# clancylian/retinaface

Hardware: NVIDIA H100
Metric: faces/sec (end-to-end detect) (higher is better)
Workload: dtype f16

## Files before the change

### retinaface_b200/csrc/engine_internal.cuh

```cuda
#pragma once
#include <algorithm>
#include <cstdarg>
#include <cstdio>
#include <cstring>
#include <functional>
#include <map>
#include <memory>
#include <string>
#include <type_traits>
#include <vector>

#include "align.cuh"
#include "common.cuh"
#include "host_copy.h"
#include "model.h"
#include "postproc.cuh"
#include "preprocess.cuh"

using namespace rf;

#define RF_STR2(x) #x
#define RF_STR(x) RF_STR2(x)

namespace rf_eng {

// ... 234 lines not shown
    virtual void heads(const HeadsNode &n) = 0;
    virtual SegOut segment(const SegNode &s, int in);
    virtual void merge_aggr(const MergeNode &m);
    virtual void ssh(const SshNode &n);
};
void walk_network(PlanOps &ops);
struct StemPack { std::vector<float> w0, wd, wp; };
StemPack pack_stem(const StemNode &n);
std::vector<float> pack_dw(const FoldedConv &dw, float scale = 1.f);
struct DwGeom { int rows, nsplit, Rmax; };
DwGeom dw_geometry(int C, int N, int IH, int IW, int S, const std::function<bool(int rows, int N, int R)> &fits);
int dw2d_tile_w(rf_handle h, int C, int oh, int ow, int nsplit);
bool aggr_fits_one_wave(rf_handle h, int fh, int fw);

constexpr int TC_SMEM_LIMIT = 200 * 1024;
template <typename T>
void build_plan(rf_handle h);
cudaError_t tc_init();
template <typename OutT>
int plan_stem_fused(Builder &B, const StemNode &n, const char *suffix, float out_scale);
int resident_ctas(rf_handle h, const void *kern, int threads, size_t smem);
struct PersistentGrid { int run, grid; };
inline PersistentGrid persistent_grid(int tiles, int resident) {
    const int run = std::max(1, (tiles + resident - 1) / std::max(resident, 1));
    return {run, (tiles + run - 1) / run};
}
int plan_pair_tc(Builder &B, const PairNode &p, int in);
void plan_conv_tc(Builder &B, const ConvNode &c);
int plan_fpn_merge_h2(Builder &B, const MergeNode &m);
template <typename T>
void plan_heads(Builder &B, const HeadsNode &n, const float scale[3], const char *prefix, bool with_heads);
std::vector<__half> pack_tc_weights(const std::vector<const FoldedConv *> &cs, std::vector<float> &bias, int &Kpad, int nsplit = 1);
void build_plan_tiles(rf_handle h);
cudaError_t tile_init();
std::string describe_chains(rf_handle h);
void comm_release(rf_handle h);
void comm_wait_in_graph(rf_handle h, const Ctx &c, int n, cudaStream_t s);
int jpeg_info(rf_handle h, const uint8_t *data, size_t len, int *w, int *hgt);
int jpeg_decode(rf_handle h, const uint8_t *const *data, const size_t *len, int n, uint8_t *const *dst, const int *w, const int *hgt, cudaStream_t s);
void jpeg_release(rf_handle h);
const char *jpeg_backend(rf_handle h);
void build_plan_i8(rf_handle h);
cudaError_t tc_init_i8();

int check_n(rf_handle h, int n);
int check_frames(rf_handle h, const char *who, const rf_yuv_frame *frames, int n, int matrix);
int check_orientations(rf_handle h, const char *who, const int *orientations, int n);
void upload_plane(rf_handle h, cudaStream_t s, uint8_t *d_dst, const uint8_t *src, size_t row_bytes, size_t pitch, int rows);
int align_setup(rf_handle h, const char *who, const rf_align_params *p, AlignArgs &a);
// ... 86 lines not shown
```

### retinaface_b200/csrc/plan_fp.cu

```cuda
#include "engine_internal.cuh"
#include "kernels_simt.cuh"
#include "stem_tc.cuh"
#include "tc_conv.cuh"
#include "tc_dwpw2d.cuh"

namespace rf_eng {

#define CK_L(...) CK(launch_k(__VA_ARGS__))

std::vector<float> pack_gemm(const std::vector<const FoldedConv *> &cs, std::vector<float> &bias) {
    const int cin = cs[0]->cin, k = cs[0]->k;
    int N = 0;
    for (auto c : cs) N += c->cout;
    std::vector<float> w((size_t)k * k * cin * N);
    bias.assign(N, 0.f);
    int n0 = 0;
    for (auto c : cs) {
        for (int o = 0; o < c->cout; o++) {
            bias[n0 + o] = c->b[o];
            for (int ci = 0; ci < cin; ci++)
                for (int t = 0; t < k * k; t++)
                    w[((size_t)t * cin + ci) * N + n0 + o] = c->w[((size_t)o * cin + ci) * k * k + t];
        }
        n0 += c->cout;
// ... 54 lines not shown
}
void launch_tc_dwpw(const TcDwArgs &a_in, int nsplit, cudaStream_t s) {
    TcDwArgs a = a_in;
    a.mul_Wp = fast_div_mul((uint32_t)a.Wp); a.mul_Hp = fast_div_mul((uint32_t)a.Hp);
    a.mul_OW = fast_div_mul((uint32_t)a.OW); a.mul_OH = fast_div_mul((uint32_t)a.OH);
    const long M = (long)a.nimg * a.OH * a.OW;
    dim3 grid((unsigned)((M + a.rows - 1) / a.rows), nsplit);
    const size_t smem = tc_dw_smem_bytes(a);
    switch (tc_n_bucket(a.N)) {
        case 32: CK_L(k_tc_dwpw_staged<32>, grid, dim3(TC_THREADS), smem, s, a); break;
        case 64: CK_L(k_tc_dwpw_staged<64>, grid, dim3(TC_THREADS), smem, s, a); break;
        case 128: CK_L(k_tc_dwpw_staged<128>, grid, dim3(TC_THREADS), smem, s, a); break;
        default: CK_L(k_tc_dwpw_staged<256>, grid, dim3(TC_THREADS), smem, s, a); break;
    }
}
static void (*dw2d_kernel(int N))(TcDw2dArgs) {
    switch (tc_n_bucket(N)) {
        case 32: return k_tc_dwpw_2d<32>;
        case 64: return k_tc_dwpw_2d<64>;
        case 128: return k_tc_dwpw_2d<128>;
        default: return k_tc_dwpw_2d<256>;
    }
}
void launch_tc_dwpw_2d(TcDw2dArgs a, int resident, cudaStream_t s) {
    const PersistentGrid pg = persistent_grid(a.tiles_x * a.tiles_y * a.nimg, resident);
    a.run = pg.run;
    CK_L(dw2d_kernel(a.N), dim3((unsigned)pg.grid), dim3(TC_THREADS), tc_dw2d_smem_bytes(a), s, a);
}

int resident_ctas(rf_handle h, const void *kern, int threads, size_t smem) {
    if (!h->on_device) return h->num_sms;
    int per_sm = 0;
    CK(cudaOccupancyMaxActiveBlocksPerMultiprocessor(&per_sm, kern, threads, smem));
    if (per_sm < 1) throw PlanFail{RF_ERR_UNSUPPORTED, fmt("a kernel with %zu bytes of dynamic shared memory does not fit an SM", smem)};
    return per_sm * h->num_sms;
}

cudaError_t tc_init() {
    cudaError_t e;
#define RF_TC_ATTR(K_) if ((e = cudaFuncSetAttribute(K_, cudaFuncAttributeMaxDynamicSharedMemorySize, TC_SMEM_LIMIT))) return e
    RF_TC_ATTR((k_tc_conv_staged<32, false>)); RF_TC_ATTR((k_tc_conv_staged<64, false>)); RF_TC_ATTR((k_tc_conv_staged<128, false>)); RF_TC_ATTR((k_tc_conv_staged<256, false>));
    RF_TC_ATTR((k_tc_conv_staged<32, true>)); RF_TC_ATTR((k_tc_conv_staged<64, true>)); RF_TC_ATTR((k_tc_conv_staged<128, true>)); RF_TC_ATTR((k_tc_conv_staged<256, true>));
    RF_TC_ATTR(k_tc_dwpw_staged<32>); RF_TC_ATTR(k_tc_dwpw_staged<64>); RF_TC_ATTR(k_tc_dwpw_staged<128>); RF_TC_ATTR(k_tc_dwpw_staged<256>);
    RF_TC_ATTR(k_tc_dwpw_2d<32>); RF_TC_ATTR(k_tc_dwpw_2d<64>); RF_TC_ATTR(k_tc_dwpw_2d<128>); RF_TC_ATTR(k_tc_dwpw_2d<256>);
#undef RF_TC_ATTR
    return cudaSuccess;
}

static std::vector<__half> make_stem_blob(const StemPack &p, const std::vector<float> &b0, const std::vector<float> &bd, const std::vector<float> &bp) {
    std::vector<__half> b0img(2 * 4 * 16 * 8, __float2half(0.f)), b1img(2 * 16 * 8, __float2half(0.f));
    for (int k = 0; k < 27; k++)
        for (int o = 0; o < 8; o++) {
            const float wv = p.w0[k * 8 + o];
            const __half hi = __float2half(wv);
            b0img[((k / 8) * 16 + o) * 8 + (k % 8)] = hi;
            b0img[((4 + k / 8) * 16 + o) * 8 + (k % 8)] = __float2half(wv - __half2float(hi));
        }
    for (int c = 0; c < 8; c++)
// ... 25 lines not shown
        TcDwArgs a{};
        a.C = C; a.Rmax = R; a.Kpad = (C + 15) / 16 * 16; a.N = Ns; a.rows = rows;
        return R <= TC_MAX_R && tc_dw_smem_bytes(a) <= (size_t)TC_SMEM_LIMIT;
    });
    if (geo.rows == 0) throw PlanFail{RF_ERR_UNSUPPORTED, fmt("layer %s (%dx%d, %d channels) does not fit shared memory", dw.name.c_str(), iw, ih, C)};
    std::vector<float> bias;
    int Kpad = 0;
    std::vector<__half> img = pack_tc_weights({&pw}, bias, Kpad, geo.nsplit);
    size_t oimg = B.add_weights_h(img), obp = B.add_weights(bias);
    int tpw = B.tensor(p.out, oh, ow_, N);
    Step s;
    s.name = fmt("tc_dw%d+pw%d_s%d_%dto%d", i, i + 1, S, C, N);
    s.in = {tin}; s.out = {tpw};
    s.flops_per_img = 2.0 * oh * ow_ * C * 9 + 2.0 * oh * ow_ * C * N;
    s.bytes_per_img = ((double)ih * iw * C + (double)oh * ow_ * N) * es;
    const int tw = dw2d_tile_w(h, C, oh, ow_, geo.nsplit);
    TcDw2dArgs g2{};
    int resident = 0;
    if (tw) {
        s.name = fmt("tc2d_dw%d+pw%d_s%d_%dto%d", i, i + 1, S, C, N);
        g2.C = C; g2.IH = ih; g2.IW = iw; g2.OH = oh; g2.OW = ow_; g2.S = S; g2.N = N;
        g2.TH = 8; g2.TW = tw;
        tc_dw2d_finish(g2);
        resident = resident_ctas(h, (const void *)dw2d_kernel(N), TC_THREADS, tc_dw2d_smem_bytes(g2));
    }
    s.launch = [=](const Run &r) {
        if (tw) {
            TcDw2dArgs a = g2;
            a.in = T_(r, tin); a.nimg = r.n;
            a.wimg = h->d_weights_h + oimg; a.bias = Wd(obp); a.dw_w = Wd(owd); a.dw_b = Wd(obd); a.out = T_(r, tpw);
            launch_tc_dwpw_2d(a, resident, r.stream);
            return;
        }
        TcDwArgs a{};
        a.in = T_(r, tin); a.C = C; a.nimg = r.n; a.IH = ih; a.IW = iw; a.OH = oh; a.OW = ow_; a.S = S;
        a.N = N / geo.nsplit; a.Ntotal = N; a.Kpad = Kpad; a.rows = geo.rows; a.Wp = iw + 2; a.Hp = ih + 1; a.Rmax = geo.Rmax;
        a.wimg = h->d_weights_h + oimg; a.bias = Wd(obp); a.dw_w = Wd(owd); a.dw_b = Wd(obd); a.out = T_(r, tpw);
        launch_tc_dwpw(a, geo.nsplit, r.stream);
    };
    B.step(std::move(s));
    return tpw;
}

void plan_conv_tc(Builder &B, const ConvNode &c) {
    rf_handle h = B.h;
    const Model &m = h->model;
// ... 273 lines not shown
```

### retinaface_b200/csrc/plan_tile.cu

```cuda
#include <cstdlib>

#include "engine_internal.cuh"
#include "tile_chain.cuh"

namespace rf_eng {

namespace {

typedef CUresult (*EncodeTiledFn)(CUtensorMap *, CUtensorMapDataType, cuuint32_t, void *, const cuuint64_t *, const cuuint64_t *,
                                  const cuuint32_t *, const cuuint32_t *, CUtensorMapInterleave, CUtensorMapSwizzle, CUtensorMapL2promotion,
                                  CUtensorMapFloatOOBfill);
EncodeTiledFn g_encode = nullptr;

constexpr int TCH_SMEM_LIMIT = 226 * 1024;

CUtensorMap make_map(const void *base, int C, int W, int H, int n, int bc, int bw, int bh, int es) {
    CUtensorMap m;
    cuuint64_t dims[4] = {(cuuint64_t)C, (cuuint64_t)W, (cuuint64_t)H, (cuuint64_t)n};
    cuuint64_t strides[3] = {(cuuint64_t)C * 2, (cuuint64_t)W * C * 2, (cuuint64_t)H * W * C * 2};
    cuuint32_t box[4] = {(cuuint32_t)bc, (cuuint32_t)bw, (cuuint32_t)bh, 1};
    cuuint32_t est[4] = {1, (cuuint32_t)es, (cuuint32_t)es, 1};
    const CUtensorMapSwizzle sw = bc * 2 == 128 ? CU_TENSOR_MAP_SWIZZLE_128B : (bc * 2 == 64 ? CU_TENSOR_MAP_SWIZZLE_64B : CU_TENSOR_MAP_SWIZZLE_32B);
    CUresult r = g_encode(&m, CU_TENSOR_MAP_DATA_TYPE_FLOAT16, 4, const_cast<void *>(base), dims, strides, box, est, CU_TENSOR_MAP_INTERLEAVE_NONE, sw,
                          CU_TENSOR_MAP_L2_PROMOTION_L2_128B, CU_TENSOR_MAP_FLOAT_OOB_FILL_NONE);
    if (r != CUDA_SUCCESS) throw PlanFail{RF_ERR_CUDA, fmt("cuTensorMapEncodeTiled failed (%d) for a %dx%dx%d tensor, box %dx%dx%d", (int)r, C, W, H, bc, bw, bh)};
    return m;
}

int round_up(int v, int a) { return (v + a - 1) / a * a; }

}

struct TileChain {
    struct LBuf {
        int C = 0;
        int halo = 0;
        bool stored = false;
        int store_tensor = -1;
        int first = 1 << 30, last = -1;
        bool is_input = false, is_merge = false;
    };
    struct LStage {
        int type = TCH_CONV, Cin = 0, N = 0, taps = 1, stride = 1, in_buf = 0;
        std::vector<int> ob_buf, ob_c16, ob_relu;
        std::vector<__half> wd_img, wp_img;
// ... 317 lines not shown
            fprintf(stderr, "TRACE %s:", c.name.c_str());
            for (unsigned i = 0; i < n; i++) fprintf(stderr, " %llu@%llu", it->second[1 + 2 * i], it->second[2 + 2 * i] - it->second[2]);
            fprintf(stderr, "\n");
        }
        memset(it->second, 0, 8 * 1024);
        a.trace = it->second;
    }
#endif
    a.warena = reinterpret_cast<const unsigned char *>(h->d_weights_h);
    a.bias = h->d_weights + c.bias_off;
    TchMaps maps;
    memset(&maps, 0, sizeof maps);
    const TchBuf &b0 = a.buf[0];
    const int bc = std::min(c.in_C, 64);
    auto T_ = [&](int id) { return r.ctx.arena + h->tensors[id].offset; };
    if (c.in_s2) maps.in = make_map(T_(c.in_tensor), c.in_C, c.in_W, c.in_H, n, bc, 2 * a.Wl, 2 * b0.nrows, 2);
    else maps.in = make_map(T_(c.in_tensor), c.in_C, c.in_W, c.in_H, n, bc, a.Wl, b0.nrows, 1);
    if (c.merge_tensor >= 0) maps.aux = make_map(T_(c.merge_tensor), 64, c.W / 2, c.H / 2, n, 64, c.W / 2 + 2, a.merge_rows, 1);
    for (int i = 0; i < c.nstores; i++) maps.st[i] = make_map(T_(c.bufs[c.store_buf_of[i]].store_tensor), c.store_C[i], c.W, c.H, n, std::min(c.store_C[i], 64), c.W, 1, 1);
    if (c.level >= 0) {
        a.head.lv = h->lv[c.level];
        a.head.pb = r.ctx.pb;
        a.head.params = r.ctx.d_params;
        a.head.net_w = h->cfg.net_w; a.head.net_h = h->cfg.net_h;
        a.head.done = r.ctx.pb.tile_done;
        a.head.expected = (c.fused_nms && !r.single) ? h->tile_expected : 0;
        for (int k = 0; k < 3; k++) a.head.blobs[k] = r.blobs ? r.blobs[3 * c.level + k] : nullptr;
    }
    const int grid = std::min(a.ntiles, h->num_sms);
    CK(launch_k(k_tile_chain<0>, dim3((unsigned)grid), dim3(TCH_THREADS), (size_t)a.smem_bytes, st, maps, a));
}

void add_chain_step(Builder &B, std::shared_ptr<TileChain> c, int lane, double bytes_per_img) {
    rf_handle h = B.h;
// ... 16 lines not shown
}

std::string describe_chains(rf_handle h) {
    std::string out;
    for (auto &cp : h->chains) {
        const TileChain &c = *cp;
        const TchArgs &a = c.args;
        out += fmt("%s: %dx%d map, TH=%d HT=%d Wl=%d, %d tiles/image, %d stages, %d MMA tiles/tile, smem %d B (%s weights), stores %d\n",
                   c.name.c_str(), c.W, c.H, a.TH, a.HT, a.Wl, a.tiles_per_img, a.nstages, c.mtiles, a.smem_bytes, a.resident ? "resident" : "streamed",
                   c.nstores);
    }
    return out;
}

cudaError_t tile_init() {
    if (!g_encode) {
        void *fn = nullptr;
        cudaDriverEntryPointQueryResult q;
        cudaError_t e = cudaGetDriverEntryPoint("cuTensorMapEncodeTiled", &fn, cudaEnableDefault, &q);
        if (e != cudaSuccess) return e;
        if (!fn) return cudaErrorNotSupported;
        g_encode = (EncodeTiledFn)fn;
    }
    return cudaFuncSetAttribute(k_tile_chain<0>, cudaFuncAttributeMaxDynamicSharedMemorySize, TCH_SMEM_LIMIT);
}

enum { TM_A = 1, TM_B = 2, TM_C = 4, TM_D = 8, TM_E = 16, TM_AGGR = 32, TM_SSH = 64, TM_HEAD = 128, TM_NMS = 256, TM_ALL = 511 };
constexpr unsigned TM_LATENCY = TM_SSH | TM_HEAD | TM_NMS;
constexpr unsigned TM_LATENCY_SMALL = TM_AGGR | TM_SSH | TM_HEAD | TM_NMS;
constexpr unsigned TM_THROUGHPUT = 0;

struct TileOps : PlanOps {
    unsigned mask;
    const bool single = env_int("RF_TILE_SINGLE", 0) != 0;
    std::shared_ptr<TileChain> ssh_chain[3];
    bool split_heads = false;
    TileOps(rf_handle h, unsigned m) : PlanOps(h), mask(m) {
        if (!(mask & TM_SSH)) mask &= ~(TM_HEAD | TM_NMS);
// ... 122 lines not shown
```

### retinaface_b200/csrc/tc_dwpw2d.cuh

```cuda
#pragma once
#include "tc_conv.cuh"

namespace rf {

struct TcDw2dArgs {
    const __half *in;
    int C, nimg, IH, IW, OH, OW, S;
    int N;
    int TH, TW;
    int tiles_x, tiles_y;
    int run;
    int PH, PW;
    uint32_t lbo_a;
    uint32_t mul_TW, mul_tiles_x, mul_tiles;
    const __half *wimg;
    const float *bias;
    const float *dw_w, *dw_b;
    __half *out;
};

inline void tc_dw2d_finish(TcDw2dArgs &a) {
    const int G = a.C >> 3;
    a.PH = (a.TH - 1) * a.S + 3;
    a.PW = (a.TW - 1) * a.S + 3;
    a.tiles_x = (a.OW + a.TW - 1) / a.TW;
    a.tiles_y = (a.OH + a.TH - 1) / a.TH;
    a.lbo_a = (uint32_t)(128 + 8 / G) * 16;
    a.mul_TW = fast_div_mul((uint32_t)a.TW);
    a.mul_tiles_x = fast_div_mul((uint32_t)a.tiles_x);
    a.mul_tiles = fast_div_mul((uint32_t)(a.tiles_x * a.tiles_y));
}
inline size_t tc_dw2d_smem_bytes(const TcDw2dArgs &a) {
    return 2 * (size_t)a.PH * a.PW * a.C * 2 + (size_t)(a.C / 8) * a.lbo_a + (size_t)a.C * a.N * 2 + 128;
}

#ifndef RF_DW2D_OCC
#define RF_DW2D_OCC 3
#endif
template <int NT>
__global__ void __launch_bounds__(TC_THREADS, RF_DW2D_OCC) k_tc_dwpw_2d(const TcDw2dArgs a) {
    extern __shared__ __align__(128) unsigned char smem[];
    __shared__ __align__(8) uint64_t bar_b;
    __shared__ float s_bias[256];
    __shared__ __align__(16) float s_dww[9 * 64];
    __shared__ __align__(16) float s_dwb[64];

    const int tid = threadIdx.x, warp = tid >> 5, lane = tid & 31;
    const int G = a.C >> 3, lg = 31 - __clz(G);
    const int PH = a.PH, PW = a.PW;
    const uint32_t lbo_a = a.lbo_a;
    const int pix = a.C * 2;
    const uint32_t stage_bytes = (uint32_t)(PH * PW * pix);
    unsigned char *sA = smem + 2 * (size_t)stage_bytes;
    unsigned char *sB = sA + (size_t)G * lbo_a;
    const int tiles = a.tiles_x * a.tiles_y;
    const int t_end = min((int)blockIdx.x * a.run + a.run, tiles * a.nimg);
    auto decode = [&](int t, int &b, int &oy0, int &ox0) {
        b = fast_div(t, a.mul_tiles);
        const int trem = t - b * tiles, ty0 = fast_div(trem, a.mul_tiles_x);
        oy0 = ty0 * a.TH; ox0 = (trem - ty0 * a.tiles_x) * a.TW;
    };

    if (tid == 0) {
        tc::mbar_init(&bar_b, 1);
        asm volatile("fence.mbarrier_init.release.cluster;" ::: "memory");
        const unsigned bytes = (unsigned)((size_t)a.C * a.N * 2);
        tc::mbar_expect_tx(&bar_b, bytes);
        tc::bulk_g2s(sB, a.wimg, bytes, &bar_b);
    }
    pdl_trigger();
    if (tid < a.N) s_bias[tid] = a.bias[tid];
    for (int i = tid; i < 9 * a.C; i += TC_THREADS) s_dww[i] = dw_weight_f16(a.dw_w[i]);
    if (tid < a.C) s_dwb[tid] = a.dw_b[tid];
    pdl_wait();
    const uint32_t sS_s = tc::smem_u32(smem);
    auto stage = [&](int t, int buf) {
        int b, oy0, ox0;
        decode(t, b, oy0, ox0);
        const int iy0 = oy0 * a.S - 1, ix0 = ox0 * a.S - 1;
        const int per_row = PW << lg;
        const int px_lo = max(0, -ix0), px_hi = min(PW, a.IW - ix0);
        const unsigned px_n = (unsigned)max(px_hi - px_lo, 0);
        for (int py = warp; py < PH; py += TC_THREADS / 32) {
            const int iy = iy0 + py;
            const bool rowok = iy >= 0 && iy < a.IH;
            const __half *src_row = a.in + (ptrdiff_t)(((b * a.IH + (rowok ? iy : 0)) * a.IW + ix0) * a.C);
            const uint32_t dst_row = sS_s + (uint32_t)buf * stage_bytes + (uint32_t)(py * PW * pix);
            const __half *zsrc = a.in;
            for (int i = lane; i < per_row; i += 32) {
                const bool ok = rowok && (unsigned)((i >> lg) - px_lo) < px_n;
                cp_async16_zfill_s(dst_row + (uint32_t)i * 16u, ok ? src_row + i * 8 : zsrc, ok);
            }
        }
        cp_async_commit();
    };
    auto stencil = [&](auto s_, const unsigned char *sS) {
        constexpr int S = decltype(s_)::value;
        const int items = a.TH * (a.TW >> 1) << lg;
        for (int it = tid; it < items; it += TC_THREADS) {
            const int g = it & (G - 1), rest = it >> lg;
            const int ty = fast_div(2 * rest, a.mul_TW), tx = 2 * rest - ty * a.TW;
            float acc[1][2][8];
            dw_bias8(acc[0][0], &s_dwb[g * 8]);
#pragma unroll
            for (int i = 0; i < 8; i++) acc[0][1][i] = acc[0][0][i];
            dw_stencil_block<S, 1, 2>(acc, sS + (ty * S * PW + tx * S) * pix + g * 16, PW * pix, pix, &s_dww[g * 8], a.C);
            unsigned char *dst = sA + (size_t)g * lbo_a + (size_t)(ty * a.TW + tx) * 16;
            *reinterpret_cast<uint4 *>(dst) = dw_relu_h8(acc[0][0]);
            *reinterpret_cast<uint4 *>(dst + 16) = dw_relu_h8(acc[0][1]);
        }
    };
    const int rows = a.TH * a.TW;
    const bool has_gemm = 64 * (warp >> 2) < rows;
    const int t_begin = (int)blockIdx.x * a.run;
    stage(t_begin, 0);
    for (int t = t_begin; t < t_end; t++) {
        const int buf = (t - t_begin) & 1;
        cp_async_wait_all();
        __syncthreads();
        if (t + 1 < t_end) stage(t + 1, buf ^ 1);
        const unsigned char *sS = smem + (size_t)buf * stage_bytes;
        if (a.S == 1) stencil(std::integral_constant<int, 1>{}, sS);
        else stencil(std::integral_constant<int, 2>{}, sS);
        tc::fence_async_smem();
        __syncthreads();
        if (!has_gemm) continue;
        tc::mbar_wait(&bar_b, 0);
        int b, oy0, ox0;
        decode(t, b, oy0, ox0);
        long orow[2];
#pragma unroll
        for (int e = 0; e < 2; e++) {
            const int r = tc_frag_row() + 8 * e;
            const int ty = fast_div(r, a.mul_TW), tx = r - ty * a.TW;
            const int oy = oy0 + ty, ox = ox0 + tx;
            orow[e] = (r < rows && oy < a.OH && ox < a.OW) ? (long)((b * a.OH + oy) * a.OW + ox) : -1;
        }
        const uint32_t a_addr = tc::smem_u32(sA) + (uint32_t)(64 * (warp >> 2)) * 16u, b_addr = tc::smem_u32(sB);
        const uint32_t lbo_b = (uint32_t)a.N * 16;
        const TcOut o{a.out, a.N, a.N, 1, nullptr, 0, 0};
        wg::for_chunks<(NT < 32 ? NT : 32)>(a.N, [&](auto nc, int n0) {
            constexpr int NC = decltype(nc)::value;
            float d[NC / 2];
            wg::fence();
            wg::mma_ss<NC>(d, wg::desc(a_addr, lbo_a, 128), wg::desc(b_addr + (uint32_t)n0 * 16u, lbo_b, 128), 0);
            for (int ks = 1; ks < (a.C >> 4); ks++) {
                const uint64_t ad = wg::desc(a_addr + (uint32_t)(2 * ks) * lbo_a, lbo_a, 128);
                const uint64_t bd = wg::desc(b_addr + (uint32_t)(2 * ks) * lbo_b + (uint32_t)n0 * 16u, lbo_b, 128);
                wg::mma_ss<NC>(d, ad, bd, 1);
            }
            wg::commit();
            wg::wait<0>();
            wg::fence_regs(d);
            tc_epilogue<NC>(d, n0, s_bias, o, orow, 0);
        });
    }
}

}
```

### retinaface_b200/csrc/tile_chain.cuh

```cuda
#pragma once
#include <cuda.h>

#include "common.cuh"
#include "postproc_dev.cuh"
#include "tc_conv.cuh"
#include "wgmma.cuh"

namespace rf {

constexpr int TCH_THREADS = 288;
constexpr int TCH_MAX_STAGES = 8;
constexpr int TCH_MAX_BUFS = 8;
constexpr int TCH_EPI_THREADS = 256;
enum { TCH_CONV = 0, TCH_DWPW = 1, TCH_HEAD = 2 };

struct TchBuf {
    int off;
    int row;
    int slabs;
    int slab_stride;
    int rows_lo;
    int nrows;
    int slack;
};
// ... 39 lines not shown
    int in_s2, plane_stride, in_C;
    unsigned in_bytes;
    int merge_C, merge_buf, merge_rows, merge_w_bias;
    unsigned merge_bytes;
    TchHead head;
};

struct TchMaps {
    CUtensorMap in;
    CUtensorMap aux;
    CUtensorMap st[3];
};

namespace tch {

__device__ __forceinline__ void tma_load_4d(uint32_t dst, const CUtensorMap *map, uint64_t *bar, int c0, int c1, int c2, int c3) {
    asm volatile("cp.async.bulk.tensor.4d.shared::cluster.global.mbarrier::complete_tx::bytes [%0], [%1, {%3, %4, %5, %6}], [%2];"
                 ::"r"(dst), "l"(map), "r"(tc::smem_u32(bar)), "r"(c0), "r"(c1), "r"(c2), "r"(c3)
                 : "memory");
}
__device__ __forceinline__ void tma_store_4d(const CUtensorMap *map, uint32_t src, int c0, int c1, int c2, int c3) {
    asm volatile("cp.async.bulk.tensor.4d.global.shared::cta.bulk_group [%0, {%2, %3, %4, %5}], [%1];"
                 ::"l"(map), "r"(src), "r"(c0), "r"(c1), "r"(c2), "r"(c3)
                 : "memory");
}
__device__ __forceinline__ void wait(uint64_t *bar, unsigned parity, unsigned *dbg, unsigned code) {
    unsigned done = 0, spins = 0;
    while (!done) {
        asm volatile(
            "{\n\t.reg .pred p;\n\t"
            "mbarrier.try_wait.parity.shared::cta.b64 p, [%1], %2;\n\t"
            "selp.u32 %0, 1, 0, p;\n\t}"
            : "=r"(done)
            : "r"(tc::smem_u32(bar)), "r"(parity)
            : "memory");
        if (!done && ++spins > (1u << 22)) {
            if (dbg) { *reinterpret_cast<volatile unsigned *>(dbg) = code | (blockIdx.x << 20); __threadfence_system(); __nanosleep(2000000); }
            __trap();
        }
    }
// ... 3 lines not shown
    __syncwarp();
}
#ifdef RF_TCH_TRACE
__device__ __forceinline__ void trace(unsigned long long *t, unsigned code) {
    if (t && blockIdx.x == 0) {
        unsigned long long now;
        asm volatile("mov.u64 %0, %%globaltimer;" : "=l"(now));
        const unsigned i = atomicAdd(reinterpret_cast<unsigned *>(t), 1u);
        if (i < 500) { t[1 + 2 * i] = code; t[2 + 2 * i] = now; }
    }
}
#define TCH_TRACE(code) tch::trace(a.trace, (code))
#else
#define TCH_TRACE(code)
#endif
__device__ __forceinline__ void bulk_commit() { asm volatile("cp.async.bulk.commit_group;" ::: "memory"); }
__device__ __forceinline__ void bulk_wait_read0() { asm volatile("cp.async.bulk.wait_group.read 0;" ::: "memory"); }
__device__ __forceinline__ void bulk_wait0() { asm volatile("cp.async.bulk.wait_group 0;" ::: "memory"); }
__device__ __forceinline__ void prefetch_map(const CUtensorMap *map) { asm volatile("prefetch.tensormap [%0];" ::"l"(map) : "memory"); }
__device__ __forceinline__ void mbar_arrive(uint64_t *bar) {
    asm volatile("mbarrier.arrive.shared::cta.b64 _, [%0];" ::"r"(tc::smem_u32(bar)) : "memory");
}
__device__ __forceinline__ void bulk_g2s_u32(uint32_t dst, const void *src, unsigned bytes, uint64_t *bar) {
    asm volatile("cp.async.bulk.shared::cluster.global.mbarrier::complete_tx::bytes [%0], [%1], %2, [%3];" ::"r"(dst), "l"(src), "r"(bytes),
                 "r"(tc::smem_u32(bar))
                 : "memory");
}
__device__ __forceinline__ void epi_bar() { asm volatile("bar.sync 1, %0;" ::"n"(TCH_EPI_THREADS) : "memory"); }
__device__ __forceinline__ uint32_t pack_h2(float a, float b) {
    __half2 h = __floats2half2_rn(a, b);
    return *reinterpret_cast<uint32_t *>(&h);
}
__device__ __forceinline__ uint32_t chunk_off(int row, int p, int j) {
    const int sh = row == 128 ? 0 : (row == 64 ? 1 : 2), m = (row >> 4) - 1;
// ... 131 lines not shown
    __syncthreads();
    if (tid == 0) TCH_TRACE(1);

    if (warp == 8) {
        if (lane == 0) {
            const unsigned bias_bytes = (unsigned)a.bias_floats * 4u;
            unsigned const_bytes = bias_bytes;
            if (a.resident) for (int s = 0; s < a.nstages; s++) const_bytes += (unsigned)(a.st[s].wd_bytes + a.st[s].wp_bytes);
            tc::mbar_expect_tx(&bar_bias, const_bytes);
            tch::bulk_g2s_u32(sbase + a.bias_smem, a.bias, bias_bytes, &bar_bias);
            if (a.resident)
                for (int s = 0; s < a.nstages; s++) {
                    if (a.st[s].wd_bytes) tch::bulk_g2s_u32(sbase + a.st[s].wd_smem, a.warena + a.st[s].wd_off, (unsigned)a.st[s].wd_bytes, &bar_bias);
                    tch::bulk_g2s_u32(sbase + a.st[s].wp_smem, a.warena + a.st[s].wp_off, (unsigned)a.st[s].wp_bytes, &bar_bias);
                }
            tch::prefetch_map(&maps.in);
            pdl_wait();
            unsigned sc = 0;
            const TchBuf &B0 = a.buf[0];
            auto store_rows = [&](const TchBuf &BS, int map, int ty, int b) {
                for (int rr = 0; rr < a.TH; rr++) {
                    const int y = ty * a.TH + rr;
                    if (y >= a.H) break;
                    for (int k = 0; k < BS.slabs; k++)
                        tch::tma_store_4d(&maps.st[map], sbase + BS.off + k * BS.slab_stride + (BS.slack + (a.HT - BS.rows_lo + rr) * Wl + 1) * BS.row, k * 64, 0, y, b);
                }
                tch::bulk_commit();
            };
            for (int tile = blockIdx.x, it = 0; tile < a.ntiles; tile += gridDim.x, it++) {
                const int b = tile / a.tiles_per_img, ty = tile - b * a.tiles_per_img;
                const int Y0 = ty * a.TH - a.HT;
                if (it > 0) { tch::wait(&bar_tile, (it - 1) & 1, a.dbg, __LINE__); tch::bulk_wait_read0(); }
                tc::mbar_expect_tx(&bar_in, a.in_bytes + a.merge_bytes);
                const int in_slabs = (a.in_C + 63) >> 6;
                if (!a.in_s2) {
                    for (int s = 0; s < in_slabs; s++)
                        tch::tma_load_4d(sbase + B0.off + s * B0.slab_stride + B0.slack * B0.row, &maps.in, &bar_in, s * 64, -1, Y0 + B0.rows_lo, b);
                } else {
                    for (int k = 0; k < 4; k++)
                        for (int s = 0; s < in_slabs; s++)
                            tch::tma_load_4d(sbase + B0.off + k * a.plane_stride + s * B0.slab_stride + B0.slack * B0.row, &maps.in, &bar_in, s * 64,
                                             -2 + (k & 1), 2 * (Y0 + a.st[0].rows_lo - 1) + (k >> 1), b);
                }
                if (a.merge_C) {
                    const TchBuf &BM = a.buf[a.merge_buf];
                    const int cy0 = ((Y0 + B0.rows_lo + 1) >> 1) - 1;
                    tch::tma_load_4d(sbase + BM.off, &maps.aux, &bar_in, 0, -1, cy0, b);
                }
                for (int s = 0; s < a.nstages; s++, sc++) {
                    const TchStage &st = a.st[s];
                    if (s > 0) {
                        tch::wait(&bar_stage, (sc - 1) & 1, a.dbg, __LINE__);
                        const TchStage &sp = a.st[s - 1];
                        if (sp.store_buf >= 0) store_rows(a.buf[sp.store_buf], sp.store_map, ty, b);
                    }
                    if (!a.resident) {
                        if (st.wd_bytes) {
                            tc::mbar_expect_tx(&bar_wd_full, (unsigned)st.wd_bytes);
                            tch::bulk_g2s_u32(sbase + a.wd_smem, a.warena + st.wd_off, (unsigned)st.wd_bytes, &bar_wd_full);
                        }
                        tc::mbar_expect_tx(&bar_wp_full, (unsigned)st.wp_bytes);
                        tch::bulk_g2s_u32(sbase + a.wp_smem, a.warena + st.wp_off, (unsigned)st.wp_bytes, &bar_wp_full);
                    }
                }
                tch::wait(&bar_stage, (sc - 1) & 1, a.dbg, __LINE__);
                {
                    const TchStage &sp = a.st[a.nstages - 1];
                    if (sp.store_buf >= 0) store_rows(a.buf[sp.store_buf], sp.store_map, ty, b);
                }
            }
            tch::bulk_wait0();
        }
    } else {
        const int wgi = warp >> 2, t4 = lane & 3;
        const int rl = 16 * (warp & 3) + (lane >> 2);
        const int etid = tid;
        const float *s_bias = reinterpret_cast<const float *>(smem + a.bias_smem);
        tch::wait_warp(&bar_bias, 0, a.dbg, __LINE__);
        pdl_wait();
        unsigned g = 0, sc = 0, wdc = 0, wpc = 0;
        for (int tile = blockIdx.x, it = 0; tile < a.ntiles; tile += gridDim.x, it++) {
            const int b = tile / a.tiles_per_img, ty = tile - b * a.tiles_per_img;
            const int Y0 = ty * a.TH - a.HT;
            tch::wait_warp(&bar_in, it & 1, a.dbg, __LINE__);
            if (lane == 0) TCH_TRACE(3);
            if (a.merge_C) {
// ... 165 lines not shown
```

Baseline: 334,000.

## Move 2-D depthwise+pointwise kernel input/output to TMA with staged output tiles

The fused 2-D depthwise+pointwise tensor-core kernel now loads its padded input tile with a TMA tensor map instead of per-thread cp.async with zero-fill, and writes output through a shared-memory staging buffer stored by TMA. A single issuer thread drives these transfers. Depthwise weights, biases and pointwise weights are packed into one constant blob that is fetched with a single bulk copy, replacing per-thread global loads. TMA helpers are moved into a shared header. The extra output staging raises shared-memory use (new 223KB limit), which can lower residency, and the path is restricted to certain output channel counts.

New measurement: 345,100 (median of 6 runs). +3.3%, better.

```diff
diff --git a/retinaface_b200/csrc/engine_internal.cuh b/retinaface_b200/csrc/engine_internal.cuh
--- a/retinaface_b200/csrc/engine_internal.cuh
+++ b/retinaface_b200/csrc/engine_internal.cuh
@@ -9,6 +9,8 @@
 #include <string>
 #include <type_traits>
 #include <vector>
+
+#include <cuda.h>
 
 #include "align.cuh"
 #include "common.cuh"
@@ -273,6 +275,7 @@
 bool aggr_fits_one_wave(rf_handle h, int fh, int fw);
 
 constexpr int TC_SMEM_LIMIT = 200 * 1024;
+constexpr int TC_DW2D_SMEM_LIMIT = 223 * 1024;
 template <typename T>
 void build_plan(rf_handle h);
 cudaError_t tc_init();
@@ -292,6 +295,7 @@
 std::vector<__half> pack_tc_weights(const std::vector<const FoldedConv *> &cs, std::vector<float> &bias, int &Kpad, int nsplit = 1);
 void build_plan_tiles(rf_handle h);
 cudaError_t tile_init();
+CUtensorMap make_map(const void *base, int C, int W, int H, int n, int bc, int bw, int bh, int es, CUtensorMapSwizzle sw);
 std::string describe_chains(rf_handle h);
 void comm_release(rf_handle h);
 void comm_wait_in_graph(rf_handle h, const Ctx &c, int n, cudaStream_t s);
diff --git a/retinaface_b200/csrc/plan_fp.cu b/retinaface_b200/csrc/plan_fp.cu
--- a/retinaface_b200/csrc/plan_fp.cu
+++ b/retinaface_b200/csrc/plan_fp.cu
@@ -92,7 +92,7 @@
         default: CK_L(k_tc_dwpw_staged<256>, grid, dim3(TC_THREADS), smem, s, a); break;
     }
 }
-static void (*dw2d_kernel(int N))(TcDw2dArgs) {
+static void (*dw2d_kernel(int N))(CUtensorMap, CUtensorMap, TcDw2dArgs) {
     switch (tc_n_bucket(N)) {
         case 32: return k_tc_dwpw_2d<32>;
         case 64: return k_tc_dwpw_2d<64>;
@@ -100,10 +100,13 @@
         default: return k_tc_dwpw_2d<256>;
     }
 }
-void launch_tc_dwpw_2d(TcDw2dArgs a, int resident, cudaStream_t s) {
+void launch_tc_dwpw_2d(TcDw2dArgs a, const __half *in, __half *out, int resident, cudaStream_t s) {
     const PersistentGrid pg = persistent_grid(a.tiles_x * a.tiles_y * a.nimg, resident);
     a.run = pg.run;
-    CK_L(dw2d_kernel(a.N), dim3((unsigned)pg.grid), dim3(TC_THREADS), tc_dw2d_smem_bytes(a), s, a);
+    const int nb = std::min(a.N, 64);
+    const CUtensorMap in_map = make_map(in, a.C, a.IW, a.IH, a.nimg, a.C, a.PW, a.PH, 1, CU_TENSOR_MAP_SWIZZLE_NONE);
+    const CUtensorMap out_map = make_map(out, a.N, a.OW, a.OH, a.nimg, nb, a.TW, a.TH, 1, tma::swizzle_for(nb * 2));
+    CK_L(dw2d_kernel(a.N), dim3((unsigned)pg.grid), dim3(TC_THREADS), tc_dw2d_smem_bytes(a), s, in_map, out_map, a);
 }
 
 int resident_ctas(rf_handle h, const void *kern, int threads, size_t smem) {
@@ -120,6 +123,8 @@
     RF_TC_ATTR((k_tc_conv_staged<32, false>)); RF_TC_ATTR((k_tc_conv_staged<64, false>)); RF_TC_ATTR((k_tc_conv_staged<128, false>)); RF_TC_ATTR((k_tc_conv_staged<256, false>));
     RF_TC_ATTR((k_tc_conv_staged<32, true>)); RF_TC_ATTR((k_tc_conv_staged<64, true>)); RF_TC_ATTR((k_tc_conv_staged<128, true>)); RF_TC_ATTR((k_tc_conv_staged<256, true>));
     RF_TC_ATTR(k_tc_dwpw_staged<32>); RF_TC_ATTR(k_tc_dwpw_staged<64>); RF_TC_ATTR(k_tc_dwpw_staged<128>); RF_TC_ATTR(k_tc_dwpw_staged<256>);
+#undef RF_TC_ATTR
+#define RF_TC_ATTR(K_) if ((e = cudaFuncSetAttribute(K_, cudaFuncAttributeMaxDynamicSharedMemorySize, TC_DW2D_SMEM_LIMIT))) return e
     RF_TC_ATTR(k_tc_dwpw_2d<32>); RF_TC_ATTR(k_tc_dwpw_2d<64>); RF_TC_ATTR(k_tc_dwpw_2d<128>); RF_TC_ATTR(k_tc_dwpw_2d<256>);
 #undef RF_TC_ATTR
     return cudaSuccess;
@@ -175,22 +180,33 @@
     s.in = {tin}; s.out = {tpw};
     s.flops_per_img = 2.0 * oh * ow_ * C * 9 + 2.0 * oh * ow_ * C * N;
     s.bytes_per_img = ((double)ih * iw * C + (double)oh * ow_ * N) * es;
-    const int tw = dw2d_tile_w(h, C, oh, ow_, geo.nsplit);
+    const int tw = tc_dw2d_store_fits(N) ? dw2d_tile_w(h, C, oh, ow_, geo.nsplit) : 0;
     TcDw2dArgs g2{};
     int resident = 0;
+    size_t oconst = 0;
     if (tw) {
         s.name = fmt("tc2d_dw%d+pw%d_s%d_%dto%d", i, i + 1, S, C, N);
         g2.C = C; g2.IH = ih; g2.IW = iw; g2.OH = oh; g2.OW = ow_; g2.S = S; g2.N = N;
         g2.TH = 8; g2.TW = tw;
         tc_dw2d_finish(g2);
+        std::vector<float> fl = pack_dw(dw);
+        for (float &v : fl) v = __half2float(__float2half_rn(v));
+        fl.insert(fl.end(), dw.b.begin(), dw.b.end());
+        fl.insert(fl.end(), bias.begin(), bias.end());
+        std::vector<__half> blob(img);
+        blob.resize(tc_dw2d_const_bytes(C, N) / 2);
+        memcpy(blob.data() + img.size(), fl.data(), fl.size() * 4);
+        oconst = B.add_weights_h(blob);
+        if (tc_dw2d_smem_bytes(g2) > (size_t)TC_DW2D_SMEM_LIMIT)
+            throw PlanFail{RF_ERR_UNSUPPORTED, fmt("layer %s (%dx%d, %d channels): the 2-D tile does not fit shared memory", dw.name.c_str(), iw, ih, C)};
         resident = resident_ctas(h, (const void *)dw2d_kernel(N), TC_THREADS, tc_dw2d_smem_bytes(g2));
     }
     s.launch = [=](const Run &r) {
         if (tw) {
             TcDw2dArgs a = g2;
-            a.in = T_(r, tin); a.nimg = r.n;
-            a.wimg = h->d_weights_h + oimg; a.bias = Wd(obp); a.dw_w = Wd(owd); a.dw_b = Wd(obd); a.out = T_(r, tpw);
-            launch_tc_dwpw_2d(a, resident, r.stream);
+            a.nimg = r.n;
+            a.consts = h->d_weights_h + oconst;
+            launch_tc_dwpw_2d(a, T_(r, tin), T_(r, tpw), resident, r.stream);
             return;
         }
         TcDwArgs a{};
diff --git a/retinaface_b200/csrc/plan_tile.cu b/retinaface_b200/csrc/plan_tile.cu
--- a/retinaface_b200/csrc/plan_tile.cu
+++ b/retinaface_b200/csrc/plan_tile.cu
@@ -7,28 +7,17 @@
 
 namespace {
 
-typedef CUresult (*EncodeTiledFn)(CUtensorMap *, CUtensorMapDataType, cuuint32_t, void *, const cuuint64_t *, const cuuint64_t *,
-                                  const cuuint32_t *, const cuuint32_t *, CUtensorMapInterleave, CUtensorMapSwizzle, CUtensorMapL2promotion,
-                                  CUtensorMapFloatOOBfill);
-EncodeTiledFn g_encode = nullptr;
-
 constexpr int TCH_SMEM_LIMIT = 226 * 1024;
 
-CUtensorMap make_map(const void *base, int C, int W, int H, int n, int bc, int bw, int bh, int es) {
+int round_up(int v, int a) { return (v + a - 1) / a * a; }
+
+}
+
+CUtensorMap make_map(const void *base, int C, int W, int H, int n, int bc, int bw, int bh, int es, CUtensorMapSwizzle sw) {
     CUtensorMap m;
-    cuuint64_t dims[4] = {(cuuint64_t)C, (cuuint64_t)W, (cuuint64_t)H, (cuuint64_t)n};
-    cuuint64_t strides[3] = {(cuuint64_t)C * 2, (cuuint64_t)W * C * 2, (cuuint64_t)H * W * C * 2};
-    cuuint32_t box[4] = {(cuuint32_t)bc, (cuuint32_t)bw, (cuuint32_t)bh, 1};
-    cuuint32_t est[4] = {1, (cuuint32_t)es, (cuuint32_t)es, 1};
-    const CUtensorMapSwizzle sw = bc * 2 == 128 ? CU_TENSOR_MAP_SWIZZLE_128B : (bc * 2 == 64 ? CU_TENSOR_MAP_SWIZZLE_64B : CU_TENSOR_MAP_SWIZZLE_32B);
-    CUresult r = g_encode(&m, CU_TENSOR_MAP_DATA_TYPE_FLOAT16, 4, const_cast<void *>(base), dims, strides, box, est, CU_TENSOR_MAP_INTERLEAVE_NONE, sw,
-                          CU_TENSOR_MAP_L2_PROMOTION_L2_128B, CU_TENSOR_MAP_FLOAT_OOB_FILL_NONE);
+    const CUresult r = tma::make_map(&m, base, C, W, H, n, bc, bw, bh, es, sw);
     if (r != CUDA_SUCCESS) throw PlanFail{RF_ERR_CUDA, fmt("cuTensorMapEncodeTiled failed (%d) for a %dx%dx%d tensor, box %dx%dx%d", (int)r, C, W, H, bc, bw, bh)};
     return m;
-}
-
-int round_up(int v, int a) { return (v + a - 1) / a * a; }
-
 }
 
 struct TileChain {
@@ -376,10 +365,14 @@
     const TchBuf &b0 = a.buf[0];
     const int bc = std::min(c.in_C, 64);
     auto T_ = [&](int id) { return r.ctx.arena + h->tensors[id].offset; };
-    if (c.in_s2) maps.in = make_map(T_(c.in_tensor), c.in_C, c.in_W, c.in_H, n, bc, 2 * a.Wl, 2 * b0.nrows, 2);
-    else maps.in = make_map(T_(c.in_tensor), c.in_C, c.in_W, c.in_H, n, bc, a.Wl, b0.nrows, 1);
-    if (c.merge_tensor >= 0) maps.aux = make_map(T_(c.merge_tensor), 64, c.W / 2, c.H / 2, n, 64, c.W / 2 + 2, a.merge_rows, 1);
-    for (int i = 0; i < c.nstores; i++) maps.st[i] = make_map(T_(c.bufs[c.store_buf_of[i]].store_tensor), c.store_C[i], c.W, c.H, n, std::min(c.store_C[i], 64), c.W, 1, 1);
+    const CUtensorMapSwizzle sw_in = tma::swizzle_for(bc * 2);
+    if (c.in_s2) maps.in = make_map(T_(c.in_tensor), c.in_C, c.in_W, c.in_H, n, bc, 2 * a.Wl, 2 * b0.nrows, 2, sw_in);
+    else maps.in = make_map(T_(c.in_tensor), c.in_C, c.in_W, c.in_H, n, bc, a.Wl, b0.nrows, 1, sw_in);
+    if (c.merge_tensor >= 0) maps.aux = make_map(T_(c.merge_tensor), 64, c.W / 2, c.H / 2, n, 64, c.W / 2 + 2, a.merge_rows, 1, CU_TENSOR_MAP_SWIZZLE_128B);
+    for (int i = 0; i < c.nstores; i++) {
+        const int sc = std::min(c.store_C[i], 64);
+        maps.st[i] = make_map(T_(c.bufs[c.store_buf_of[i]].store_tensor), c.store_C[i], c.W, c.H, n, sc, c.W, 1, 1, tma::swizzle_for(sc * 2));
+    }
     if (c.level >= 0) {
         a.head.lv = h->lv[c.level];
         a.head.pb = r.ctx.pb;
@@ -426,14 +419,7 @@
 }
 
 cudaError_t tile_init() {
-    if (!g_encode) {
-        void *fn = nullptr;
-        cudaDriverEntryPointQueryResult q;
-        cudaError_t e = cudaGetDriverEntryPoint("cuTensorMapEncodeTiled", &fn, cudaEnableDefault, &q);
-        if (e != cudaSuccess) return e;
-        if (!fn) return cudaErrorNotSupported;
-        g_encode = (EncodeTiledFn)fn;
-    }
+    if (cudaError_t e = tma::init()) return e;
     return cudaFuncSetAttribute(k_tile_chain<0>, cudaFuncAttributeMaxDynamicSharedMemorySize, TCH_SMEM_LIMIT);
 }
 
diff --git a/retinaface_b200/csrc/tc_dwpw2d.cuh b/retinaface_b200/csrc/tc_dwpw2d.cuh
--- a/retinaface_b200/csrc/tc_dwpw2d.cuh
+++ b/retinaface_b200/csrc/tc_dwpw2d.cuh
@@ -1,23 +1,23 @@
 #pragma once
 #include "tc_conv.cuh"
+#include "tma.cuh"
 
 namespace rf {
 
 struct TcDw2dArgs {
-    const __half *in;
     int C, nimg, IH, IW, OH, OW, S;
     int N;
     int TH, TW;
     int tiles_x, tiles_y;
     int run;
     int PH, PW;
+    uint32_t stage_bytes;
+    uint32_t out_slab;
     uint32_t lbo_a;
     uint32_t mul_TW, mul_tiles_x, mul_tiles;
-    const __half *wimg;
-    const float *bias;
-    const float *dw_w, *dw_b;
-    __half *out;
+    const __half *consts;
 };
+__host__ __device__ inline size_t tc_dw2d_const_bytes(int C, int N) { return (size_t)C * N * 2 + (size_t)(10 * C + N) * 4; }
 
 inline void tc_dw2d_finish(TcDw2dArgs &a) {
     const int G = a.C >> 3;
@@ -25,74 +25,78 @@
     a.PW = (a.TW - 1) * a.S + 3;
     a.tiles_x = (a.OW + a.TW - 1) / a.TW;
     a.tiles_y = (a.OH + a.TH - 1) / a.TH;
+    a.stage_bytes = (uint32_t)(a.PH * a.PW * a.C * 2 + 127) / 128 * 128;
+    a.out_slab = (uint32_t)(a.TH * a.TW * (a.N < 64 ? a.N : 64) * 2 + 1023) / 1024 * 1024;
     a.lbo_a = (uint32_t)(128 + 8 / G) * 16;
     a.mul_TW = fast_div_mul((uint32_t)a.TW);
     a.mul_tiles_x = fast_div_mul((uint32_t)a.tiles_x);
     a.mul_tiles = fast_div_mul((uint32_t)(a.tiles_x * a.tiles_y));
 }
+inline bool tc_dw2d_store_fits(int N) { return N == 16 || N == 32 || N == 64 || (N % 64 == 0 && N <= 256); }
 inline size_t tc_dw2d_smem_bytes(const TcDw2dArgs &a) {
-    return 2 * (size_t)a.PH * a.PW * a.C * 2 + (size_t)(a.C / 8) * a.lbo_a + (size_t)a.C * a.N * 2 + 128;
+    const int slabs = a.N > 64 ? a.N / 64 : 1;
+    return (size_t)slabs * a.out_slab + 2 * (size_t)a.stage_bytes + (size_t)(a.C / 8) * a.lbo_a + tc_dw2d_const_bytes(a.C, a.N) + 1024;
 }
 
 #ifndef RF_DW2D_OCC
 #define RF_DW2D_OCC 3
 #endif
 template <int NT>
-__global__ void __launch_bounds__(TC_THREADS, RF_DW2D_OCC) k_tc_dwpw_2d(const TcDw2dArgs a) {
-    extern __shared__ __align__(128) unsigned char smem[];
-    __shared__ __align__(8) uint64_t bar_b;
-    __shared__ float s_bias[256];
-    __shared__ __align__(16) float s_dww[9 * 64];
-    __shared__ __align__(16) float s_dwb[64];
+__global__ void __launch_bounds__(TC_THREADS, RF_DW2D_OCC) k_tc_dwpw_2d(const __grid_constant__ CUtensorMap in_map,
+                                                                      const __grid_constant__ CUtensorMap out_map, const TcDw2dArgs a) {
+    extern __shared__ __align__(128) unsigned char smem_raw[];
+    __shared__ __align__(8) uint64_t bar_b, bar_in[2];
 
-    const int tid = threadIdx.x, warp = tid >> 5, lane = tid & 31;
+    const int tid = threadIdx.x;
+    constexpr int ISSUER = TC_THREADS - 32;
     const int G = a.C >> 3, lg = 31 - __clz(G);
     const int PH = a.PH, PW = a.PW;
     const uint32_t lbo_a = a.lbo_a;
     const int pix = a.C * 2;
-    const uint32_t stage_bytes = (uint32_t)(PH * PW * pix);
+    const uint32_t stage_bytes = a.stage_bytes;
+    const int NB = a.N < 64 ? a.N : 64, slabs = a.N / NB;
+    const uint32_t raw_s = tc::smem_u32(smem_raw), base_s = (raw_s + 1023u) & ~1023u;
+    unsigned char *sOut = smem_raw + (base_s - raw_s);
+    unsigned char *smem = sOut + (size_t)slabs * a.out_slab;
     unsigned char *sA = smem + 2 * (size_t)stage_bytes;
     unsigned char *sB = sA + (size_t)G * lbo_a;
+    const float *s_dww = reinterpret_cast<const float *>(sB + (size_t)a.C * a.N * 2);
+    const float *s_dwb = s_dww + 9 * a.C, *s_bias = s_dwb + a.C;
     const int tiles = a.tiles_x * a.tiles_y;
-    const int t_end = min((int)blockIdx.x * a.run + a.run, tiles * a.nimg);
+    const int t_begin = (int)blockIdx.x * a.run;
+    const int t_end = min(t_begin + a.run, tiles * a.nimg);
     auto decode = [&](int t, int &b, int &oy0, int &ox0) {
         b = fast_div(t, a.mul_tiles);
         const int trem = t - b * tiles, ty0 = fast_div(trem, a.mul_tiles_x);
         oy0 = ty0 * a.TH; ox0 = (trem - ty0 * a.tiles_x) * a.TW;
     };
 
-    if (tid == 0) {
+    if (tid == ISSUER) {
         tc::mbar_init(&bar_b, 1);
+        tc::mbar_init(&bar_in[0], 1);
+        tc::mbar_init(&bar_in[1], 1);
         asm volatile("fence.mbarrier_init.release.cluster;" ::: "memory");
-        const unsigned bytes = (unsigned)((size_t)a.C * a.N * 2);
+        const unsigned bytes = (unsigned)tc_dw2d_const_bytes(a.C, a.N);
         tc::mbar_expect_tx(&bar_b, bytes);
-        tc::bulk_g2s(sB, a.wimg, bytes, &bar_b);
+        tc::bulk_g2s(sB, a.consts, bytes, &bar_b);
+        tma::prefetch_map(&in_map);
+        tma::prefetch_map(&out_map);
     }
     pdl_trigger();
-    if (tid < a.N) s_bias[tid] = a.bias[tid];
-    for (int i = tid; i < 9 * a.C; i += TC_THREADS) s_dww[i] = dw_weight_f16(a.dw_w[i]);
-    if (tid < a.C) s_dwb[tid] = a.dw_b[tid];
     pdl_wait();
     const uint32_t sS_s = tc::smem_u32(smem);
-    auto stage = [&](int t, int buf) {
+    auto load = [&](int t, int buf) {
         int b, oy0, ox0;
         decode(t, b, oy0, ox0);
-        const int iy0 = oy0 * a.S - 1, ix0 = ox0 * a.S - 1;
-        const int per_row = PW << lg;
-        const int px_lo = max(0, -ix0), px_hi = min(PW, a.IW - ix0);
-        const unsigned px_n = (unsigned)max(px_hi - px_lo, 0);
-        for (int py = warp; py < PH; py += TC_THREADS / 32) {
-            const int iy = iy0 + py;
-            const bool rowok = iy >= 0 && iy < a.IH;
-            const __half *src_row = a.in + (ptrdiff_t)(((b * a.IH + (rowok ? iy : 0)) * a.IW + ix0) * a.C);
-            const uint32_t dst_row = sS_s + (uint32_t)buf * stage_bytes + (uint32_t)(py * PW * pix);
-            const __half *zsrc = a.in;
-            for (int i = lane; i < per_row; i += 32) {
-                const bool ok = rowok && (unsigned)((i >> lg) - px_lo) < px_n;
-                cp_async16_zfill_s(dst_row + (uint32_t)i * 16u, ok ? src_row + i * 8 : zsrc, ok);
-            }
-        }
-        cp_async_commit();
+        tc::mbar_expect_tx(&bar_in[buf], (unsigned)(PH * PW * pix));
+        tma::load_4d(sS_s + (uint32_t)buf * stage_bytes, &in_map, &bar_in[buf], 0, ox0 * a.S - 1, oy0 * a.S - 1, b);
+    };
+    const uint32_t sOut_s = tc::smem_u32(sOut);
+    auto store = [&](int t) {
+        int b, oy0, ox0;
+        decode(t, b, oy0, ox0);
+        for (int k = 0; k < slabs; k++) tma::store_4d(&out_map, sOut_s + (uint32_t)k * a.out_slab, k * NB, ox0, oy0, b);
+        tma::bulk_commit();
     };
     auto stencil = [&](auto s_, const unsigned char *sS) {
         constexpr int S = decltype(s_)::value;
@@ -111,34 +115,28 @@
         }
     };
     const int rows = a.TH * a.TW;
-    const bool has_gemm = 64 * (warp >> 2) < rows;
-    const int t_begin = (int)blockIdx.x * a.run;
-    stage(t_begin, 0);
+    const bool has_gemm = 64 * (tid >> 7) < rows;
+    if (tid == ISSUER) load(t_begin, 0);
     for (int t = t_begin; t < t_end; t++) {
-        const int buf = (t - t_begin) & 1;
-        cp_async_wait_all();
+        const int j = t - t_begin, buf = j & 1;
         __syncthreads();
-        if (t + 1 < t_end) stage(t + 1, buf ^ 1);
+        if (tid == ISSUER) {
+            if (t > t_begin) store(t - 1);
+            if (t + 1 < t_end) load(t + 1, buf ^ 1);
+        }
+        tc::mbar_wait(&bar_in[buf], (unsigned)(j >> 1) & 1u);
+        tc::mbar_wait(&bar_b, 0);
         const unsigned char *sS = smem + (size_t)buf * stage_bytes;
         if (a.S == 1) stencil(std::integral_constant<int, 1>{}, sS);
         else stencil(std::integral_constant<int, 2>{}, sS);
         tc::fence_async_smem();
+        if (tid == ISSUER) tma::bulk_wait_read0();
         __syncthreads();
         if (!has_gemm) continue;
-        tc::mbar_wait(&bar_b, 0);
-        int b, oy0, ox0;
-        decode(t, b, oy0, ox0);
-        long orow[2];
-#pragma unroll
-        for (int e = 0; e < 2; e++) {
-            const int r = tc_frag_row() + 8 * e;
-            const int ty = fast_div(r, a.mul_TW), tx = r - ty * a.TW;
-            const int oy = oy0 + ty, ox = ox0 + tx;
-            orow[e] = (r < rows && oy < a.OH && ox < a.OW) ? (long)((b * a.OH + oy) * a.OW + ox) : -1;
-        }
-        const uint32_t a_addr = tc::smem_u32(sA) + (uint32_t)(64 * (warp >> 2)) * 16u, b_addr = tc::smem_u32(sB);
+        const int r0 = tc_frag_row(), c2 = 2 * (tid & 3);
+        const uint32_t rb = (uint32_t)NB * 2;
+        const uint32_t a_addr = tc::smem_u32(sA) + (uint32_t)(64 * (tid >> 7)) * 16u, b_addr = tc::smem_u32(sB);
         const uint32_t lbo_b = (uint32_t)a.N * 16;
-        const TcOut o{a.out, a.N, a.N, 1, nullptr, 0, 0};
         wg::for_chunks<(NT < 32 ? NT : 32)>(a.N, [&](auto nc, int n0) {
             constexpr int NC = decltype(nc)::value;
             float d[NC / 2];
@@ -152,8 +150,25 @@
             wg::commit();
             wg::wait<0>();
             wg::fence_regs(d);
-            tc_epilogue<NC>(d, n0, s_bias, o, orow, 0);
+#pragma unroll
+            for (int e = 0; e < 2; e++) {
+                const int r = r0 + 8 * e;
+                if (r >= rows) continue;
+#pragma unroll
+                for (int i = 0; i < NC / 8; i++) {
+                    const int n = n0 + 8 * i + c2;
+                    const uint32_t off = (uint32_t)(n >> 6) * a.out_slab + tma::swz((uint32_t)r * rb + (uint32_t)(n & 63) * 2u, rb);
+                    const float f0 = fmaxf(d[4 * i + 2 * e] + s_bias[n], 0.f), f1 = fmaxf(d[4 * i + 2 * e + 1] + s_bias[n + 1], 0.f);
+                    *reinterpret_cast<__half2 *>(sOut + off) = __floats2half2_rn(f0, f1);
+                }
+            }
         });
+        tc::fence_async_smem();
+    }
+    __syncthreads();
+    if (tid == ISSUER) {
+        store(t_end - 1);
+        tma::bulk_wait_read0();
     }
 }
 
diff --git a/retinaface_b200/csrc/tile_chain.cuh b/retinaface_b200/csrc/tile_chain.cuh
--- a/retinaface_b200/csrc/tile_chain.cuh
+++ b/retinaface_b200/csrc/tile_chain.cuh
@@ -4,6 +4,7 @@
 #include "common.cuh"
 #include "postproc_dev.cuh"
 #include "tc_conv.cuh"
+#include "tma.cuh"
 #include "wgmma.cuh"
 
 namespace rf {
@@ -77,16 +78,6 @@
 
 namespace tch {
 
-__device__ __forceinline__ void tma_load_4d(uint32_t dst, const CUtensorMap *map, uint64_t *bar, int c0, int c1, int c2, int c3) {
-    asm volatile("cp.async.bulk.tensor.4d.shared::cluster.global.mbarrier::complete_tx::bytes [%0], [%1, {%3, %4, %5, %6}], [%2];"
-                 ::"r"(dst), "l"(map), "r"(tc::smem_u32(bar)), "r"(c0), "r"(c1), "r"(c2), "r"(c3)
-                 : "memory");
-}
-__device__ __forceinline__ void tma_store_4d(const CUtensorMap *map, uint32_t src, int c0, int c1, int c2, int c3) {
-    asm volatile("cp.async.bulk.tensor.4d.global.shared::cta.bulk_group [%0, {%2, %3, %4, %5}], [%1];"
-                 ::"l"(map), "r"(src), "r"(c0), "r"(c1), "r"(c2), "r"(c3)
-                 : "memory");
-}
 __device__ __forceinline__ void wait(uint64_t *bar, unsigned parity, unsigned *dbg, unsigned code) {
     unsigned done = 0, spins = 0;
     while (!done) {
@@ -120,10 +111,6 @@
 #else
 #define TCH_TRACE(code)
 #endif
-__device__ __forceinline__ void bulk_commit() { asm volatile("cp.async.bulk.commit_group;" ::: "memory"); }
-__device__ __forceinline__ void bulk_wait_read0() { asm volatile("cp.async.bulk.wait_group.read 0;" ::: "memory"); }
-__device__ __forceinline__ void bulk_wait0() { asm volatile("cp.async.bulk.wait_group 0;" ::: "memory"); }
-__device__ __forceinline__ void prefetch_map(const CUtensorMap *map) { asm volatile("prefetch.tensormap [%0];" ::"l"(map) : "memory"); }
 __device__ __forceinline__ void mbar_arrive(uint64_t *bar) {
     asm volatile("mbarrier.arrive.shared::cta.b64 _, [%0];" ::"r"(tc::smem_u32(bar)) : "memory");
 }
@@ -285,7 +272,7 @@
                     if (a.st[s].wd_bytes) tch::bulk_g2s_u32(sbase + a.st[s].wd_smem, a.warena + a.st[s].wd_off, (unsigned)a.st[s].wd_bytes, &bar_bias);
                     tch::bulk_g2s_u32(sbase + a.st[s].wp_smem, a.warena + a.st[s].wp_off, (unsigned)a.st[s].wp_bytes, &bar_bias);
                 }
-            tch::prefetch_map(&maps.in);
+            tma::prefetch_map(&maps.in);
             pdl_wait();
             unsigned sc = 0;
             const TchBuf &B0 = a.buf[0];
@@ -294,29 +281,29 @@
                     const int y = ty * a.TH + rr;
                     if (y >= a.H) break;
                     for (int k = 0; k < BS.slabs; k++)
-                        tch::tma_store_4d(&maps.st[map], sbase + BS.off + k * BS.slab_stride + (BS.slack + (a.HT - BS.rows_lo + rr) * Wl + 1) * BS.row, k * 64, 0, y, b);
-                }
-                tch::bulk_commit();
+                        tma::store_4d(&maps.st[map], sbase + BS.off + k * BS.slab_stride + (BS.slack + (a.HT - BS.rows_lo + rr) * Wl + 1) * BS.row, k * 64, 0, y, b);
+                }
+                tma::bulk_commit();
             };
             for (int tile = blockIdx.x, it = 0; tile < a.ntiles; tile += gridDim.x, it++) {
                 const int b = tile / a.tiles_per_img, ty = tile - b * a.tiles_per_img;
                 const int Y0 = ty * a.TH - a.HT;
-                if (it > 0) { tch::wait(&bar_tile, (it - 1) & 1, a.dbg, __LINE__); tch::bulk_wait_read0(); }
+                if (it > 0) { tch::wait(&bar_tile, (it - 1) & 1, a.dbg, __LINE__); tma::bulk_wait_read0(); }
                 tc::mbar_expect_tx(&bar_in, a.in_bytes + a.merge_bytes);
                 const int in_slabs = (a.in_C + 63) >> 6;
                 if (!a.in_s2) {
                     for (int s = 0; s < in_slabs; s++)
-                        tch::tma_load_4d(sbase + B0.off + s * B0.slab_stride + B0.slack * B0.row, &maps.in, &bar_in, s * 64, -1, Y0 + B0.rows_lo, b);
+                        tma::load_4d(sbase + B0.off + s * B0.slab_stride + B0.slack * B0.row, &maps.in, &bar_in, s * 64, -1, Y0 + B0.rows_lo, b);
                 } else {
                     for (int k = 0; k < 4; k++)
                         for (int s = 0; s < in_slabs; s++)
-                            tch::tma_load_4d(sbase + B0.off + k * a.plane_stride + s * B0.slab_stride + B0.slack * B0.row, &maps.in, &bar_in, s * 64,
+                            tma::load_4d(sbase + B0.off + k * a.plane_stride + s * B0.slab_stride + B0.slack * B0.row, &maps.in, &bar_in, s * 64,
                                              -2 + (k & 1), 2 * (Y0 + a.st[0].rows_lo - 1) + (k >> 1), b);
                 }
                 if (a.merge_C) {
                     const TchBuf &BM = a.buf[a.merge_buf];
                     const int cy0 = ((Y0 + B0.rows_lo + 1) >> 1) - 1;
-                    tch::tma_load_4d(sbase + BM.off, &maps.aux, &bar_in, 0, -1, cy0, b);
+                    tma::load_4d(sbase + BM.off, &maps.aux, &bar_in, 0, -1, cy0, b);
                 }
                 for (int s = 0; s < a.nstages; s++, sc++) {
                     const TchStage &st = a.st[s];
@@ -340,7 +327,7 @@
                     if (sp.store_buf >= 0) store_rows(a.buf[sp.store_buf], sp.store_map, ty, b);
                 }
             }
-            tch::bulk_wait0();
+            tma::bulk_wait0();
         }
     } else {
         const int wgi = warp >> 2, t4 = lane & 3;
diff --git a/retinaface_b200/csrc/tma.cuh b/retinaface_b200/csrc/tma.cuh
--- /dev/null
+++ b/retinaface_b200/csrc/tma.cuh
@@ -0,0 +1,58 @@
+#pragma once
+#include <cuda.h>
+#include <cuda_runtime.h>
+
+#include <cstdint>
+
+namespace rf {
+namespace tma {
+
+typedef CUresult (*EncodeTiledFn)(CUtensorMap *, CUtensorMapDataType, cuuint32_t, void *, const cuuint64_t *, const cuuint64_t *,
+                                  const cuuint32_t *, const cuuint32_t *, CUtensorMapInterleave, CUtensorMapSwizzle, CUtensorMapL2promotion,
+                                  CUtensorMapFloatOOBfill);
+inline EncodeTiledFn g_encode = nullptr;
+
+inline cudaError_t init() {
+    if (g_encode) return cudaSuccess;
+    void *fn = nullptr;
+    cudaDriverEntryPointQueryResult q;
+    cudaError_t e = cudaGetDriverEntryPoint("cuTensorMapEncodeTiled", &fn, cudaEnableDefault, &q);
+    if (e != cudaSuccess) return e;
+    if (!fn) return cudaErrorNotSupported;
+    g_encode = (EncodeTiledFn)fn;
+    return cudaSuccess;
+}
+
+inline CUtensorMapSwizzle swizzle_for(int row_bytes) {
+    return row_bytes == 128 ? CU_TENSOR_MAP_SWIZZLE_128B : row_bytes == 64 ? CU_TENSOR_MAP_SWIZZLE_64B
+                                                       : row_bytes == 32 ? CU_TENSOR_MAP_SWIZZLE_32B : CU_TENSOR_MAP_SWIZZLE_NONE;
+}
+
+inline CUresult make_map(CUtensorMap *m, const void *base, int C, int W, int H, int n, int bc, int bw, int bh, int es, CUtensorMapSwizzle sw) {
+    cuuint64_t dims[4] = {(cuuint64_t)C, (cuuint64_t)W, (cuuint64_t)H, (cuuint64_t)n};
+    cuuint64_t strides[3] = {(cuuint64_t)C * 2, (cuuint64_t)W * C * 2, (cuuint64_t)H * W * C * 2};
+    cuuint32_t box[4] = {(cuuint32_t)bc, (cuuint32_t)bw, (cuuint32_t)bh, 1};
+    cuuint32_t est[4] = {1, (cuuint32_t)es, (cuuint32_t)es, 1};
+    if (!g_encode) return CUDA_ERROR_NOT_INITIALIZED;
+    return g_encode(m, CU_TENSOR_MAP_DATA_TYPE_FLOAT16, 4, const_cast<void *>(base), dims, strides, box, est, CU_TENSOR_MAP_INTERLEAVE_NONE, sw,
+                    CU_TENSOR_MAP_L2_PROMOTION_L2_128B, CU_TENSOR_MAP_FLOAT_OOB_FILL_NONE);
+}
+
+__device__ __forceinline__ void load_4d(uint32_t dst, const CUtensorMap *map, uint64_t *bar, int c0, int c1, int c2, int c3) {
+    asm volatile("cp.async.bulk.tensor.4d.shared::cluster.global.mbarrier::complete_tx::bytes [%0], [%1, {%3, %4, %5, %6}], [%2];"
+                 ::"r"(dst), "l"(map), "r"((uint32_t)__cvta_generic_to_shared(bar)), "r"(c0), "r"(c1), "r"(c2), "r"(c3)
+                 : "memory");
+}
+__device__ __forceinline__ void store_4d(const CUtensorMap *map, uint32_t src, int c0, int c1, int c2, int c3) {
+    asm volatile("cp.async.bulk.tensor.4d.global.shared::cta.bulk_group [%0, {%2, %3, %4, %5}], [%1];"
+                 ::"l"(map), "r"(src), "r"(c0), "r"(c1), "r"(c2), "r"(c3)
+                 : "memory");
+}
+__device__ __forceinline__ void bulk_commit() { asm volatile("cp.async.bulk.commit_group;" ::: "memory"); }
+__device__ __forceinline__ void bulk_wait_read0() { asm volatile("cp.async.bulk.wait_group.read 0;" ::: "memory"); }
+__device__ __forceinline__ void bulk_wait0() { asm volatile("cp.async.bulk.wait_group 0;" ::: "memory"); }
+__device__ __forceinline__ void prefetch_map(const CUtensorMap *map) { asm volatile("prefetch.tensormap [%0];" ::"l"(map) : "memory"); }
+__device__ __forceinline__ uint32_t swz(uint32_t off, uint32_t row_bytes) { return off ^ (((off >> 7) & ((row_bytes >> 4) - 1)) << 4); }
+
+}
+}
```
